# NVlabs/UnseenObjectClustering

Measured on AMD Instinct MI355X. Metric: frames/sec at 640x480 RGB-D, two-stage clustering, higher is better.
Workload: dtype f32; 1 GPU; configs[3] frames: full two-stage (crop-and-refine) segmentation of single 640x480 RGB-D frames; throughput schedule 3 streams x 4-frame launch sets (one frame at a time: `latency`); frame=640x480, seeds=100, iters=10, crop=224, total_frames=513, frames_per_gpu=513, collective=False, frames_in_flight_per_gpu=12, streams_per_gpu=3, frames_per_launch=4

## Files before the change

include/uoc_hip.h:

```cpp
#ifndef UOC_HIP_H
#define UOC_HIP_H

#include <stddef.h>
#include <stdint.h>

#ifdef __cplusplus
extern "C" {
#endif

#define UOC_OK 0
#define UOC_EINVAL (-22)
#define UOC_ENOMEM (-12)
#define UOC_EHIP (-5)
#define UOC_ENOENT (-2)
#define UOC_ETIMEDOUT (-110)

#define UOC_EMBED_DIM 64
#define UOC_MAX_SEEDS 128
#define UOC_METRIC_COSINE 0
#define UOC_METRIC_EUCLIDEAN 1

int uoc_version(void);
int uoc_is_dev_build(void);
unsigned long long uoc_config_fingerprint(void);
// ... 32 lines not shown
size_t uoc_ms_workspace_bytes_wide(int batch, int n, int m, int halves);
int uoc_ms_cluster_wide(const float *d_X, int halves, int batch, int n, int m, float kappa, int iters, float epsilon,
                        const int32_t *d_first_index, int32_t *d_labels, int32_t *d_indices, float *d_Z_out,
                        int32_t *d_seed_labels_out, void *d_ws, size_t ws_bytes, void *stream);

int uoc_ms_select_seeds_ex(const float *d_X, int batch, int n, int m, int num_init, const int32_t *d_first_index,
                           float *d_seeds, int32_t *d_indices, int metric, void *d_ws, size_t ws_bytes, void *stream);
int uoc_ms_hill_climb_ex(const float *d_X, int batch, int n, float *d_Z, int m, float kappa, int iters, int metric,
                         void *d_ws, size_t ws_bytes, void *stream);
int uoc_ms_seed_components_ex(const float *d_Z, int batch, int m, float epsilon, int metric, int32_t *d_seed_labels,
                              int32_t *d_num_unique, void *stream);
int uoc_ms_assign_ex(const float *d_X, int batch, int n, const float *d_Z, const int32_t *d_seed_labels,
                     const int32_t *d_num_unique, int m, int metric, int32_t *d_labels, int32_t *d_closest, void *d_ws,
                     size_t ws_bytes, void *stream);
int uoc_ms_cluster_ex(const float *d_X, int batch, int n, int m, float kappa, int iters, float epsilon, int metric,
                      const int32_t *d_first_index, int32_t *d_labels, int32_t *d_indices, float *d_Z_out,
                      int32_t *d_seed_labels_out, void *d_ws, size_t ws_bytes, void *stream);
int uoc_ms_cluster_wide_ex(const float *d_X, int halves, int batch, int n, int m, float kappa, int iters, float epsilon,
                           int metric, const int32_t *d_first_index, int32_t *d_labels, int32_t *d_indices, float *d_Z_out,
                           int32_t *d_seed_labels_out, void *d_ws, size_t ws_bytes, void *stream);


typedef struct uoc_net uoc_net;

enum { UOC_NET_RGBD_ADD = 0, UOC_NET_COLOR = 1, UOC_NET_DEPTH = 2, UOC_NET_RGBD_EARLY = 3, UOC_NET_RGBD_CAT = 4 };

int uoc_net_create(uoc_net **out);
int uoc_net_create_mode(uoc_net **out, int mode);
int uoc_net_embed_dim(const uoc_net *net);
int uoc_net_destroy(uoc_net *net);
int uoc_net_load_param(uoc_net *net, const char *name, const float *host_data, size_t numel);
int uoc_net_finalize(uoc_net *net);
size_t uoc_net_workspace_bytes(const uoc_net *net, int B, int H, int W);
int uoc_net_set_split_precision(uoc_net *net, int on);
int uoc_net_forward(uoc_net *net, const float *d_rgb, const float *d_xyz, int B, int H, int W, float *d_embed,
                    void *d_ws, size_t ws_bytes, void *stream);

#define UOC_CONV_DIRECT 0
#define UOC_CONV_WINOGRAD4 4
#define UOC_CONV_WINOGRAD4_BF16X3 5
int uoc_conv2d_nhwc(const float *d_in, const float *d_w, const float *d_bias, const float *d_res, float *d_out,
                    int G, int B, int H, int W, int Cin, int Cout, int K, int stride, int dil, int pad, int relu,
                    void *stream);
int uoc_conv2d_nhwc_algo(const float *d_in, const float *d_w, const float *d_bias, const float *d_res, float *d_out,
                         int G, int B, int H, int W, int Cin, int Cout, int K, int stride, int dil, int pad, int relu,
                         int algo, void *stream);

int uoc_conv2d_tile_list(int algo, int32_t *out_pairs, int cap);
int uoc_conv2d_nhwc_tile(const float *d_in, const float *d_w, const float *d_bias, const float *d_res, float *d_out,
                         int G, int B, int H, int W, int Cin, int Cout, int K, int stride, int dil, int pad, int relu,
                         int algo, void *stream, int cfg, int bm);
int uoc_conv2d_tile_choice(int G, int B, int H, int W, int Cin, int Cout, int K, int stride, int dil, int algo,
                           int32_t *cfg, int32_t *bm, int32_t *family_bm);
int uoc_net_stem(const float *d_nchw, const float *h_w, const float *h_bias, const float *d_res, int G, int B, int H,
                 int W, int relu, float *d_out, void *stream);
int uoc_maxpool3x3s2_nhwc(const float *d_in, float *d_out, int n_img, int H, int W, int C, void *stream);
int uoc_head(const float *d_fa, const float *d_fb, float *d_embed, int B, int h, int w, int H, int W, int cat,
             void *stream);


typedef struct uoc_roi_table {
  int32_t K;
  int32_t label[128];
  int32_t box[128][4];
} uoc_roi_table;

size_t uoc_roi_workspace_bytes(void);

int uoc_prep_rgbd(const uint8_t *d_bgr, const uint16_t *d_depth_mm, int H, int W, float fx, float fy, float px,
                  float py, float mean_b, float mean_g, float mean_r, float *d_image, float *d_xyz, void *stream);

int uoc_filter_labels_depth(int32_t *d_labels, const float *d_z, long z_batch_stride, int B, int H, int W,
                            float threshold, void *d_ws, size_t ws_bytes, void *stream);

int uoc_roi_build(int32_t *d_labels, const float *d_z, int H, int W, float threshold, float pad_fraction,
                  uoc_roi_table *d_table, void *d_ws, size_t ws_bytes, void *stream);

int uoc_roi_crop(const float *d_rgb, const float *d_xyz, const int32_t *d_labels, int H, int W,
                 const uoc_roi_table *d_table, int K, int S, float *d_rgb_crops, float *d_xyz_crops,
                 float *d_mask_crops, void *stream);

int uoc_roi_match_stats(const int32_t *d_labels_crop, const float *d_mask_crops, const float *d_xyz_crops, int K,
                        int S, int32_t *d_keep, float *d_meanz, void *d_ws, size_t ws_bytes, void *stream);

int uoc_roi_paste(const int32_t *d_labels_crop, const uoc_roi_table *d_table, const int32_t *d_map,
                  const int32_t *d_order, int K, int S, int H, int W, int32_t *d_refined, void *stream);

int uoc_roi_match(const int32_t *d_labels_crop, const float *d_mask_crops, const float *d_xyz_crops,
                  const uoc_roi_table *d_table, int K, int S, int H, int W, int32_t *d_refined, int32_t *d_keep,
                  int32_t *d_plan, int32_t *d_status, void *d_ws, size_t ws_bytes, void *stream);

int uoc_labels_to_u8(const int32_t *d_labels, long n, uint8_t *d_out, int32_t *d_top, void *stream);


typedef struct uoc_eval_tables {
  int32_t cont[128 * 128];
  int32_t prec_tp[128 * 128];
  int32_t rec_tp[128 * 128];
  int32_t bnd_pred[128];
  int32_t bnd_gt[128];
  int32_t bad_label;
} uoc_eval_tables;

size_t uoc_eval_workspace_bytes(int H, int W);
int uoc_eval_pair_stats(const int32_t *d_pred, const int32_t *d_gt, int H, int W, int radius, uoc_eval_tables *d_tables,
                        void *d_ws, size_t ws_bytes, void *stream);
// ... 207 lines not shown
```

unseenobjectclustering_amd/_native.py:

```python
from __future__ import annotations

import ctypes
import os
from ctypes import c_char_p, c_float, c_int, c_int32, c_size_t, c_void_p, POINTER

from .build import LIB_PATH

_lib = None


class NativeError(RuntimeError):
    pass


def _declare(lib):
    P = c_void_p
    lib.uoc_version.restype = c_int
    lib.uoc_is_dev_build.argtypes = []
    lib.uoc_is_dev_build.restype = c_int
    lib.uoc_config_fingerprint.argtypes = []
    lib.uoc_config_fingerprint.restype = ctypes.c_ulonglong
    lib.uoc_shutdown.restype = c_int
    lib.uoc_reload_env.argtypes = []
    lib.uoc_reload_env.restype = c_int
    lib.uoc_shutdown.argtypes = []
    lib.uoc_last_error.restype = c_char_p
    lib.uoc_ms_set_persistent_fps.argtypes = [c_int]
    lib.uoc_ms_set_persistent_fps.restype = c_int
    lib.uoc_ms_set_stream_ordering.argtypes = [c_int]
    lib.uoc_ms_set_stream_ordering.restype = c_int
    lib.uoc_ms_fps_fallbacks.argtypes = []
    lib.uoc_ms_fps_fallbacks.restype = c_int
    lib.uoc_ms_workspace_bytes.restype = c_size_t
    lib.uoc_ms_workspace_bytes.argtypes = [c_int, c_int, c_int]
    lib.uoc_ms_select_seeds.argtypes = [P, c_int, c_int, c_int, P, P, P, P, c_size_t, P]
    lib.uoc_ms_select_seeds_from.argtypes = [P, c_int, c_int, c_int, c_int, P, P, P, P, c_size_t, P]
    lib.uoc_ms_hill_climb.argtypes = [P, c_int, c_int, P, c_int, c_float, c_int, P, c_size_t, P]
    lib.uoc_ms_seed_components.argtypes = [P, c_int, c_int, c_float, P, P, P]
    lib.uoc_ms_assign.argtypes = [P, c_int, c_int, P, P, P, c_int, P, P, P, c_size_t, P]
    lib.uoc_ms_cluster.argtypes = [P, c_int, c_int, c_int, c_float, c_int, c_float, P, P, P, P, P, P, c_size_t, P]
    lib.uoc_ms_check.argtypes = [P]
    lib.uoc_ms_check.restype = c_int
    lib.uoc_ms_workspace_bytes_wide.restype = c_size_t
    lib.uoc_ms_workspace_bytes_wide.argtypes = [c_int, c_int, c_int, c_int]
    lib.uoc_ms_cluster_wide.argtypes = [P, c_int, c_int, c_int, c_int, c_float, c_int, c_float, P, P, P, P, P, P, c_size_t, P]
    lib.uoc_ms_cluster_wide.restype = c_int
    lib.uoc_ms_select_seeds_ex.argtypes = [P, c_int, c_int, c_int, c_int, P, P, P, c_int, P, c_size_t, P]
    lib.uoc_ms_hill_climb_ex.argtypes = [P, c_int, c_int, P, c_int, c_float, c_int, c_int, P, c_size_t, P]
    lib.uoc_ms_seed_components_ex.argtypes = [P, c_int, c_int, c_float, c_int, P, P, P]
    lib.uoc_ms_assign_ex.argtypes = [P, c_int, c_int, P, P, P, c_int, c_int, P, P, P, c_size_t, P]
    lib.uoc_ms_cluster_ex.argtypes = [P, c_int, c_int, c_int, c_float, c_int, c_float, c_int, P, P, P, P, P, P, c_size_t, P]
    lib.uoc_ms_cluster_wide_ex.argtypes = [P, c_int, c_int, c_int, c_int, c_float, c_int, c_float, c_int, P, P, P, P, P, P,
                                           c_size_t, P]
    for name in METRIC_SYMBOLS:
        getattr(lib, name).restype = c_int
    lib.uoc_net_embed_dim.argtypes = [P]
    lib.uoc_net_embed_dim.restype = c_int
    lib.uoc_net_create.argtypes = [POINTER(P)]
    lib.uoc_net_create_mode.argtypes = [POINTER(P), c_int]
    lib.uoc_net_destroy.argtypes = [P]
    lib.uoc_net_load_param.argtypes = [P, c_char_p, P, c_size_t]
    lib.uoc_net_finalize.argtypes = [P]
    lib.uoc_net_workspace_bytes.restype = c_size_t
    lib.uoc_net_workspace_bytes.argtypes = [P, c_int, c_int, c_int]
    lib.uoc_net_forward.argtypes = [P, P, P, c_int, c_int, c_int, P, P, c_size_t, P]
    lib.uoc_net_set_split_precision.argtypes = [P, c_int]
    lib.uoc_net_set_split_precision.restype = c_int
    lib.uoc_conv2d_nhwc.argtypes = [P, P, P, P, P] + [c_int] * 11 + [P]
    lib.uoc_conv2d_nhwc_algo.argtypes = [P, P, P, P, P] + [c_int] * 12 + [P]
    lib.uoc_conv2d_nhwc_algo.restype = c_int
    lib.uoc_conv2d_tile_list.argtypes = [c_int, P, c_int]
    lib.uoc_conv2d_nhwc_tile.argtypes = [P, P, P, P, P] + [c_int] * 12 + [P, c_int, c_int]
    lib.uoc_conv2d_tile_choice.argtypes = [c_int] * 10 + [P, P, P]
    lib.uoc_net_stem.argtypes = [P, P, P, P] + [c_int] * 5 + [P, P]
    lib.uoc_maxpool3x3s2_nhwc.argtypes = [P, P] + [c_int] * 4 + [P]
    lib.uoc_head.argtypes = [P, P, P] + [c_int] * 6 + [P]
    for name in TILE_SYMBOLS:
        getattr(lib, name).restype = c_int
    for name in ("uoc_net_create", "uoc_net_create_mode", "uoc_net_destroy", "uoc_net_load_param", "uoc_net_finalize", "uoc_net_forward",
                 "uoc_conv2d_nhwc"):
        getattr(lib, name).restype = c_int
    lib.uoc_eval_workspace_bytes.restype = c_size_t
    lib.uoc_eval_workspace_bytes.argtypes = [c_int, c_int]
    lib.uoc_eval_pair_stats.argtypes = [P, P, c_int, c_int, c_int, P, P, c_size_t, P]
    lib.uoc_eval_pair_stats.restype = c_int
    lib.uoc_roi_workspace_bytes.restype = c_size_t
    lib.uoc_roi_workspace_bytes.argtypes = []
    lib.uoc_prep_rgbd.argtypes = [P, P, c_int, c_int] + [c_float] * 7 + [P, P, P]
    lib.uoc_prep_rgbd.restype = c_int
    lib.uoc_filter_labels_depth.argtypes = [P, P, ctypes.c_long, c_int, c_int, c_int, c_float, P, c_size_t, P]
    lib.uoc_roi_build.argtypes = [P, P, c_int, c_int, c_float, c_float, P, P, c_size_t, P]
    lib.uoc_roi_crop.argtypes = [P, P, P, c_int, c_int, P, c_int, c_int, P, P, P, P]
    lib.uoc_roi_match_stats.argtypes = [P, P, P, c_int, c_int, P, P, P, c_size_t, P]
    lib.uoc_roi_paste.argtypes = [P, P, P, P, c_int, c_int, c_int, c_int, P, P]
    lib.uoc_labels_to_u8.argtypes = [P, ctypes.c_long, P, P, P]
    lib.uoc_roi_match.argtypes = [P, P, P, P, c_int, c_int, c_int, c_int, P, P, P, P, P, c_size_t, P]
    for name in ("uoc_filter_labels_depth", "uoc_roi_build", "uoc_roi_crop", "uoc_roi_match_stats", "uoc_roi_paste", "uoc_labels_to_u8", "uoc_roi_match"):
        getattr(lib, name).restype = c_int
    lib.uoc_objects_workspace_bytes.argtypes = [c_int, c_int, c_int]
    lib.uoc_objects_workspace_bytes.restype = c_size_t
    lib.uoc_objects.argtypes = [P, P, P, c_int, c_int, c_int, c_int, c_int, P, P, P, P, ctypes.c_long, P, P, c_size_t, P]
    lib.uoc_objects.restype = c_int
    lib.uoc_track_state_bytes.argtypes = [c_int, c_int, c_int]
    lib.uoc_track_state_bytes.restype = c_size_t
    lib.uoc_track_workspace_bytes.argtypes = [c_int]
    lib.uoc_track_workspace_bytes.restype = c_size_t
    lib.uoc_track_reset.argtypes = [P, c_int, c_int, c_int, c_int, P]
    lib.uoc_track_reset.restype = c_int
    lib.uoc_track_step.argtypes = [P, c_int, c_int, c_int, c_int, c_int, P, P, P, P, P, c_size_t, P]
    lib.uoc_track_step.restype = c_int
    lib.uoc_cc_workspace_bytes.argtypes = [c_int, c_int, c_int]
    lib.uoc_cc_workspace_bytes.restype = c_size_t
    lib.uoc_cc_split.argtypes = [P, c_int, c_int, c_int, c_int, c_int, c_int, P, P, P, P, c_size_t, P]
    lib.uoc_cc_split.restype = c_int
    lib.uoc_plane_workspace_bytes.argtypes = [c_int, c_int, c_int, c_int]
    lib.uoc_plane_workspace_bytes.restype = c_size_t
    lib.uoc_support_plane.argtypes = [P, P, c_int, c_int, c_int, c_int, c_int, ctypes.c_uint32, P, P, P, P, c_size_t, P]
    lib.uoc_support_plane.restype = c_int
    lib.uoc_planes_workspace_bytes.argtypes = [c_int, c_int, c_int, c_int, c_int]
    lib.uoc_planes_workspace_bytes.restype = c_size_t
    lib.uoc_support_planes.argtypes = [P, P] + [c_int] * 8 + [ctypes.c_uint32, P, P, P, P, P, P, c_size_t, P]
    lib.uoc_support_planes.restype = c_int
    lib.uoc_relations_workspace_bytes.argtypes = [c_int, c_int, c_int]
    lib.uoc_relations_workspace_bytes.restype = c_size_t
    lib.uoc_relations.argtypes = [P, P, c_int, c_int, c_int, c_int, c_int, c_int, P, P, P, c_size_t, P]
    lib.uoc_relations.restype = c_int
    lib.uoc_placement_workspace_bytes.argtypes = [c_int, c_int, c_int, c_int]
    lib.uoc_placement_workspace_bytes.restype = c_size_t
    lib.uoc_placement.argtypes = [P, P, P] + [c_int] * 9 + [P, c_int, P, P, P, P, P, P, P, c_size_t, P]
    lib.uoc_placement.restype = c_int
    lib.uoc_grasp_workspace_bytes.argtypes = [c_int, c_int, c_int, c_int]
    lib.uoc_grasp_workspace_bytes.restype = c_size_t
    lib.uoc_grasp.argtypes = [P, P, c_int, c_int, P] + [c_int] * 7 + [P, P, P, c_size_t, P]
    lib.uoc_grasp.restype = c_int
    lib.uoc_elevation_workspace_bytes.argtypes = [c_int, c_int, c_int, c_int]
    lib.uoc_elevation_workspace_bytes.restype = c_size_t
    lib.uoc_elevation.argtypes = [P, P, P] + [c_int] * 8 + [P, c_int] + [P] * 9 + [c_size_t, P]
    lib.uoc_elevation.restype = c_int
    lib.uoc_footprint_workspace_bytes.argtypes = [c_int, c_int, c_int, c_int]
    lib.uoc_footprint_workspace_bytes.restype = c_size_t
    lib.uoc_footprint.argtypes = [P, P, P, P, c_int, c_int, P, c_int, P, c_int, c_int, P, P, P, P, c_size_t, P]
    lib.uoc_footprint.restype = c_int
    lib.uoc_routes_workspace_bytes.argtypes = [c_int, c_int, c_int]
    lib.uoc_routes_workspace_bytes.restype = c_size_t
    lib.uoc_routes.argtypes = [P, P, P, c_int, c_int, P, c_int, c_int, c_int, P, P, P, P, c_size_t, P]
    lib.uoc_routes.restype = c_int
    lib.uoc_ms_confidence_workspace_bytes.argtypes = [c_int, c_int, c_int, c_int]
    lib.uoc_ms_confidence_workspace_bytes.restype = c_size_t
    lib.uoc_ms_confidence.argtypes = [P, c_int, c_int, c_int, P, P, P, c_int, c_int, P, P, P, P, P, P, c_size_t, P]
    lib.uoc_ms_confidence.restype = c_int
    lib.uoc_conf_paste.argtypes = [P, P, P, P, c_int, c_int, c_int, c_int, P, P]
    lib.uoc_conf_paste.restype = c_int
    lib.uoc_conf_objects.argtypes = [P, P, c_int, c_int, c_int, c_int, P, P]
    lib.uoc_conf_objects.restype = c_int
    lib.uoc_normals_workspace_bytes.argtypes = [c_int, c_int, c_int]
    lib.uoc_normals_workspace_bytes.restype = c_size_t
    lib.uoc_normals.argtypes = [P, P, P] + [c_int] * 7 + [P, c_int, c_int, c_int, P, P, P, P, c_size_t, P]
    lib.uoc_normals.restype = c_int
    lib.uoc_lzf_decompress.argtypes = [P, c_size_t, P, c_size_t]
    lib.uoc_lzf_decompress.restype = ctypes.c_long
    lib.uoc_prof_enable.argtypes = [c_int]
    lib.uoc_prof_reset.argtypes = []
    lib.uoc_prof_report.argtypes = [ctypes.c_char_p, c_size_t]
    for name in ("uoc_prof_enable", "uoc_prof_reset", "uoc_prof_report"):
        getattr(lib, name).restype = c_int
    for name in ("uoc_ms_select_seeds", "uoc_ms_select_seeds_from", "uoc_ms_hill_climb", "uoc_ms_seed_components", "uoc_ms_assign",
                 "uoc_ms_cluster"):
        getattr(lib, name).restype = c_int


METRIC_COSINE = 0
METRIC_EUCLIDEAN = 1
METRICS = {"cosine": METRIC_COSINE, "euclidean": METRIC_EUCLIDEAN}
METRIC_SYMBOLS = ("uoc_ms_select_seeds_ex", "uoc_ms_hill_climb_ex", "uoc_ms_seed_components_ex", "uoc_ms_assign_ex",
                  "uoc_ms_cluster_ex", "uoc_ms_cluster_wide_ex")


TILE_SYMBOLS = ("uoc_conv2d_tile_list", "uoc_conv2d_nhwc_tile", "uoc_conv2d_tile_choice", "uoc_net_stem",
                "uoc_maxpool3x3s2_nhwc", "uoc_head")


def metric_code(metric) -> int:
    if metric not in METRICS:
        raise NotImplementedError(f"metric={metric!r}: only 'cosine' and 'euclidean' are implemented on gfx950")
    return METRICS[metric]


EXPORTED_SYMBOLS = (
    "uoc_version", "uoc_is_dev_build", "uoc_config_fingerprint", "uoc_shutdown", "uoc_last_error", "uoc_reload_env", "uoc_ms_set_persistent_fps", "uoc_ms_set_stream_ordering", "uoc_ms_fps_fallbacks", "uoc_ms_check", "uoc_ms_workspace_bytes", "uoc_ms_select_seeds", "uoc_ms_select_seeds_from", "uoc_ms_hill_climb",
    "uoc_ms_seed_components", "uoc_ms_assign", "uoc_ms_cluster", "uoc_ms_workspace_bytes_wide", "uoc_ms_cluster_wide",
) + METRIC_SYMBOLS + (
    "uoc_net_embed_dim",
    "uoc_net_create", "uoc_net_create_mode", "uoc_net_destroy", "uoc_net_load_param", "uoc_net_finalize", "uoc_net_workspace_bytes",
    "uoc_net_forward", "uoc_net_set_split_precision", "uoc_conv2d_nhwc", "uoc_conv2d_nhwc_algo",
) + TILE_SYMBOLS + (
    "uoc_roi_workspace_bytes", "uoc_prep_rgbd", "uoc_filter_labels_depth", "uoc_roi_build", "uoc_roi_crop", "uoc_roi_match_stats",
    "uoc_roi_paste", "uoc_roi_match", "uoc_labels_to_u8", "uoc_eval_workspace_bytes", "uoc_eval_pair_stats", "uoc_objects_workspace_bytes", "uoc_objects",
    "uoc_track_state_bytes", "uoc_track_workspace_bytes", "uoc_track_reset", "uoc_track_step",
    "uoc_cc_workspace_bytes", "uoc_cc_split", "uoc_plane_workspace_bytes", "uoc_support_plane",
    "uoc_planes_workspace_bytes", "uoc_support_planes",
    "uoc_relations_workspace_bytes", "uoc_relations", "uoc_placement_workspace_bytes", "uoc_placement",
    "uoc_grasp_workspace_bytes", "uoc_grasp", "uoc_elevation_workspace_bytes", "uoc_elevation",
    "uoc_footprint_workspace_bytes", "uoc_footprint", "uoc_routes_workspace_bytes", "uoc_routes",
    "uoc_ms_confidence_workspace_bytes", "uoc_ms_confidence", "uoc_conf_paste", "uoc_conf_objects",
    "uoc_normals_workspace_bytes", "uoc_normals", "uoc_lzf_decompress", "uoc_prof_enable", "uoc_prof_reset", "uoc_prof_report",
)


class RoiTable(ctypes.Structure):
    _fields_ = [("K", c_int32), ("label", c_int32 * 128), ("box", (c_int32 * 4) * 128)]


ROI_TABLE_BYTES = ctypes.sizeof(RoiTable)


class UocObject(ctypes.Structure):
    _fields_ = [("pixels", c_int32), ("count", c_int32), ("box", c_int32 * 4), ("centroid", c_float * 3), ("cov", c_float * 6),
                ("aabb_min", c_float * 3), ("aabb_max", c_float * 3), ("eig", c_float * 3), ("axes", c_float * 9),
                ("obb_center", c_float * 3), ("obb_half", c_float * 3), ("offset", c_int32), ("kept", c_int32)]


OBJECT_BYTES = ctypes.sizeof(UocObject)


class UocPlane(ctypes.Structure):
    _fields_ = [("found", c_int32), ("candidates", c_int32), ("inliers", c_int32), ("hyp", c_int32), ("normal", c_float * 3),
                ("d", c_float), ("centroid", c_float * 3), ("eig", c_float * 3), ("rms", c_float), ("u", c_float * 3),
                ("v", c_float * 3)]


class UocPlaneObject(ctypes.Structure):
    _fields_ = [("count", c_int32), ("height_min", c_float), ("height_max", c_float), ("foot", c_float * 2),
# ... 173 lines not shown
```

unseenobjectclustering_amd/csrc/conv.h:

```cpp
#pragma once
#include "common.h"

namespace uoc {

struct ConvParams {
  const float *in;
  const float *w;
  const float *bias;
  const float *res;
  float *out;
  int G, B, H, W, Cin, Ho, Wo, Cout;
  int KH, KW, stride, dil, pad, relu;
  int stem;
  int tune = 1;
  int prof_kc = -1;
  double prof_flops = 0.0;
  int prof_tag[4] = {0, 0, 0, 0};
};

int launch_conv(const ConvParams &p, hipStream_t st);
int conv_tile_list(int *out_pairs, int cap);
int conv_tile_choice(const ConvParams &p, int *cfg, int *bm, int *fam_bm);
int launch_conv_tile(const ConvParams &p, hipStream_t st, int cfg, int bm);

struct W4Tile {
  int bm, bn;
};
int wino4_tile_list(bool split, int *out_pairs, int cap);
void wino4_tile_choice(bool split, int NT, int Cout, int planes, int *bn, int *bm);
int wino4_split_tile_list(int *out_pairs, int cap);
void wino4_split_tile_choice(int NT, int Cout, int planes, int *bn, int *bm);
void wino4_pick_tile(const int (*tiles)[2], int n, int NT, int Cout, int planes, int &bm, int &bn);
int wino4_plane_grid(int NT, int Cout, int planes, int bm, int bn);

bool wino4_eligible(const ConvParams &p);
bool wino4_channels_ok(int Cin, int Cout);
size_t wino4_ws_floats(int G, int B, int H, int W, int d, int Cin, int Cout);
int wino4_num_tiles(int B, int H, int W, int d);
int launch_wino4_weights(const float *w, float *U, int G, int Cout, int Cin, hipStream_t st);
int launch_wino4_conv(const ConvParams &p, const float *U, float *ws, hipStream_t st, const unsigned short *U3 = nullptr,
                      const W4Tile *tile = nullptr);
int launch_wino4_split_weights(const float *U, unsigned short *U3, int G, int Cout, int Cin, hipStream_t st);
int launch_wino4_slice_split(const ConvParams &p0, int Bg, int b0, const unsigned short *U3, float *ws, hipStream_t st,
                             const W4Tile *tile = nullptr);
struct Wino4Geom;
int w4_stage_output(const ConvParams &p, const Wino4Geom &geo, const float *Mw, hipStream_t st);
long wino4_elem_blocks(long items);
int launch_nchw3_to_nhwc4(const float *in, float *out, int B, int H, int W, hipStream_t st);
int launch_maxpool3x3s2(const float *in, float *out, int n_img, int H, int W, int C, int Ho, int Wo, hipStream_t st);
int launch_head(const float *fa, const float *fb, float *embed, int B, int h, int w, int H, int W, int cat,
                hipStream_t st);

}
```

unseenobjectclustering_amd/csrc/net.hip:

```cpp
#include <map>
#include <mutex>
#include <string>
#include <vector>

#include "conv.h"

#include <stdlib.h>

namespace uoc {

struct ConvLayer {
  std::string conv, bn;
  int Cin, Cout, K, stride, dil, pad, relu;
  bool has_bn, has_bias, stem;
  float *d_w = nullptr, *d_b = nullptr;
  float *d_U4 = nullptr;
  unsigned short *d_U3 = nullptr;
  size_t w_per_group = 0;
};

struct Block {
  int conv1, conv2, down;
};

// ... 352 lines not shown
    if (int rc = run_conv(G, c2, tmp, res, y, B, ho, wo, ho, wo, st, w.wino, n->split)) return rc;
    cur = (cur + 3) & 3;
    h = ho;
    wd = wo;
  }
  if (int rc = run_conv(G, n->layers[n->fc], w.buf[cur], nullptr, w.fc, B, h, wd, h, wd, st)) return rc;
  return launch_head(w.fc, G == 2 ? w.fc + (size_t)B * h * wd * 64 : nullptr, d_embed, B, h, wd, H, W,
                     n->mode == UOC_NET_RGBD_CAT, st);
}

static ConvParams entry_params(int G, int B, int H, int W, int Cin, int Cout, int K, int stride, int dil, int pad, int relu) {
  ConvParams p;
  p.tune = 0;
  p.in = p.w = p.bias = p.res = nullptr;
  p.out = nullptr;
  p.G = G;
  p.B = B;
  p.H = H;
  p.W = W;
  p.Cin = Cin;
  p.Cout = Cout;
  p.KH = p.KW = K;
  p.stride = stride;
  p.dil = dil;
  p.pad = pad;
  p.relu = relu;
  p.stem = 0;
  p.Ho = (H + 2 * pad - dil * (K - 1) - 1) / stride + 1;
  p.Wo = (W + 2 * pad - dil * (K - 1) - 1) / stride + 1;
  return p;
}

static int conv2d_entry(const float *d_in, const float *d_w, const float *d_bias, const float *d_res, float *d_out, int G,
                        int B, int H, int W, int Cin, int Cout, int K, int stride, int dil, int pad, int relu, int algo,
                        void *stream, const int *tile) {
  UOC_REQUIRE(K == 1 || K == 3, "K=%d (only 1 or 3)", K);
  UOC_REQUIRE(G >= 1 && B >= 1 && H >= 1 && W >= 1 && Cin >= 1 && Cout >= 1 && stride >= 1 && dil >= 1 && pad >= 0,
              "conv2d: bad shape");
  UOC_REQUIRE(d_res == nullptr || d_res != d_out, "conv2d: the residual must not alias the output");
  ConvParams p = entry_params(G, B, H, W, Cin, Cout, K, stride, dil, pad, relu);
  p.in = d_in;
  p.w = d_w;
  p.bias = d_bias;
  p.res = d_res;
  p.out = d_out;
  hipStream_t st = (hipStream_t)stream;
  if (algo == UOC_CONV_DIRECT) return tile ? launch_conv_tile(p, st, tile[0], tile[1]) : launch_conv(p, st);
  const W4Tile w4tile = {tile ? tile[1] : 0, tile ? tile[0] : 0};
  const W4Tile *wt = tile ? &w4tile : nullptr;
  static std::mutex mu;
  std::lock_guard<std::mutex> lock(mu);
  if (algo == UOC_CONV_WINOGRAD4 || algo == UOC_CONV_WINOGRAD4_BF16X3) {
    UOC_REQUIRE(wino4_eligible(p), "conv2d: shape not eligible for Winograd F(4x4,3x3)");
    if (tile) {
      int pairs[2 * 32];
      const int n = wino4_tile_list(algo == UOC_CONV_WINOGRAD4_BF16X3, pairs, 32);
      bool listed = false;
      for (int i = 0; i < n && i < 32; ++i) listed = listed || (pairs[2 * i] == tile[0] && pairs[2 * i + 1] == tile[1]);
      UOC_REQUIRE(listed, "conv2d tile: the plane GEMM has no tile BN=%d BM=%d", tile[0], tile[1]);
      UOC_REQUIRE(Cout % tile[0] == 0, "conv2d tile: Cout=%d is not a multiple of BN=%d", Cout, tile[0]);
    }
    static float *U4 = nullptr, *ws4 = nullptr;
    static unsigned short *U3 = nullptr;
    static size_t ucap4 = 0, wcap4 = 0, ucap3 = 0;
    const size_t un = (size_t)G * 36 * Cout * Cin, wn = wino4_ws_floats(G, B, H, W, dil, Cin, Cout);
    if (un > ucap4) {
      if (U4) (void)hipFree(U4);
      UOC_HIP_CHECK(hipMalloc(&U4, un * sizeof(float)));
      ucap4 = un;
    }
    if (wn > wcap4) {
      if (ws4) (void)hipFree(ws4);
      UOC_HIP_CHECK(hipMalloc(&ws4, wn * sizeof(float)));
      wcap4 = wn;
    }
    if (int rc = launch_wino4_weights(d_w, U4, G, Cout, Cin, st)) return rc;
    if (algo == UOC_CONV_WINOGRAD4_BF16X3) {
      if (3 * un > ucap3) {
        if (U3) (void)hipFree(U3);
        UOC_HIP_CHECK(hipMalloc(&U3, 3 * un * sizeof(unsigned short)));
        ucap3 = 3 * un;
      }
      if (int rc = launch_wino4_split_weights(U4, U3, G, Cout, Cin, st)) return rc;
      return launch_wino4_conv(p, U4, ws4, st, U3, wt);
    }
    return launch_wino4_conv(p, U4, ws4, st, nullptr, wt);
  }
  set_error("conv2d: unknown algorithm %d", algo);
  return UOC_EINVAL;
}

int uoc_conv2d_nhwc_algo(const float *d_in, const float *d_w, const float *d_bias, const float *d_res, float *d_out, int G,
                         int B, int H, int W, int Cin, int Cout, int K, int stride, int dil, int pad, int relu, int algo,
                         void *stream) {
  return conv2d_entry(d_in, d_w, d_bias, d_res, d_out, G, B, H, W, Cin, Cout, K, stride, dil, pad, relu, algo, stream, nullptr);
}

int uoc_conv2d_nhwc_tile(const float *d_in, const float *d_w, const float *d_bias, const float *d_res, float *d_out, int G,
                         int B, int H, int W, int Cin, int Cout, int K, int stride, int dil, int pad, int relu, int algo,
                         void *stream, int cfg, int bm) {
  UOC_REQUIRE(d_in && d_w && d_out, "conv2d tile: null pointer");
  const int tile[2] = {cfg, bm};
  return conv2d_entry(d_in, d_w, d_bias, d_res, d_out, G, B, H, W, Cin, Cout, K, stride, dil, pad, relu, algo, stream, tile);
}

int uoc_conv2d_tile_list(int algo, int32_t *out_pairs, int cap) {
  UOC_REQUIRE(cap >= 0 && (out_pairs || cap == 0), "tile list: null array");
  if (algo == UOC_CONV_DIRECT) return conv_tile_list(out_pairs, cap);
  if (algo == UOC_CONV_WINOGRAD4 || algo == UOC_CONV_WINOGRAD4_BF16X3)
    return wino4_tile_list(algo == UOC_CONV_WINOGRAD4_BF16X3, out_pairs, cap);
  set_error("tile list: unknown algorithm %d", algo);
  return UOC_EINVAL;
}

int uoc_conv2d_tile_choice(int G, int B, int H, int W, int Cin, int Cout, int K, int stride, int dil, int algo, int32_t *cfg,
                           int32_t *bm, int32_t *family_bm) {
  UOC_REQUIRE(cfg && bm, "tile choice: null pointer");
  UOC_REQUIRE(K == 1 || K == 3, "K=%d (only 1 or 3)", K);
  UOC_REQUIRE(G >= 1 && B >= 1 && H >= 1 && W >= 1 && Cin >= 1 && Cout >= 1 && stride >= 1 && dil >= 1, "tile choice: bad shape");
  const ConvParams p = entry_params(G, B, H, W, Cin, Cout, K, stride, dil, K == 3 ? dil : 0, 0);
  if (algo == UOC_CONV_DIRECT) return conv_tile_choice(p, cfg, bm, family_bm);
  if (algo == UOC_CONV_WINOGRAD4 || algo == UOC_CONV_WINOGRAD4_BF16X3) {
    UOC_REQUIRE(wino4_eligible(p), "tile choice: shape not eligible for Winograd F(4x4,3x3)");
    int bn_ = 0, bm_ = 0;
    wino4_tile_choice(algo == UOC_CONV_WINOGRAD4_BF16X3, wino4_num_tiles(B, H, W, dil), Cout, 36 * G, &bn_, &bm_);
    *cfg = bn_;
    *bm = bm_;
    return UOC_OK;
  }
  set_error("tile choice: unknown algorithm %d", algo);
  return UOC_EINVAL;
}

int uoc_net_stem(const float *d_nchw, const float *h_w, const float *h_bias, const float *d_res, int G, int B, int H, int W,
                 int relu, float *d_out, void *stream) {
  UOC_REQUIRE(d_nchw && h_w && d_out, "stem: null pointer");
  UOC_REQUIRE(G >= 1 && B >= 1 && H >= 1 && W >= 1, "stem: bad shape");
  UOC_REQUIRE(d_res == nullptr || d_res != d_out, "stem: the residual must not alias the output");
  UOC_REQUIRE((long)G * B * H * W * 4 < (1l << 31), "stem: input too large");
  hipStream_t st = (hipStream_t)stream;
  const size_t wpg = (size_t)7 * 64 * 32;
  std::vector<float> hw((size_t)G * wpg, 0.f), hb((size_t)G * 64, 0.f);
  const std::vector<double> one(64, 1.0);
  for (int g = 0; g < G; ++g) relayout_weights(h_w + (size_t)g * 64 * 3 * 49, one.data(), 64, 3, 7, true, wpg, hw.data() + g * wpg);
  if (h_bias) hb.assign(h_bias, h_bias + (size_t)G * 64);
  float *d_w = nullptr, *d_b = nullptr, *d_in4 = nullptr;
  int rc = UOC_OK;
  auto run = [&]() -> int {
    UOC_HIP_CHECK(hipMalloc(&d_w, hw.size() * sizeof(float)));
    UOC_HIP_CHECK(hipMalloc(&d_b, hb.size() * sizeof(float)));
    UOC_HIP_CHECK(hipMalloc(&d_in4, (size_t)G * B * H * W * 4 * sizeof(float)));
    UOC_HIP_CHECK(hipMemcpyAsync(d_w, hw.data(), hw.size() * sizeof(float), hipMemcpyHostToDevice, st));
    UOC_HIP_CHECK(hipMemcpyAsync(d_b, hb.data(), hb.size() * sizeof(float), hipMemcpyHostToDevice, st));
    if (int r = launch_nchw3_to_nhwc4(d_nchw, d_in4, G * B, H, W, st)) return r;
    ConvLayer L;
    L.Cin = 3;
// ... 46 lines not shown
```

unseenobjectclustering_amd/csrc/wino4.hip:

```cpp
#include "conv.h"
#include "dma.h"
#include "prof.h"
#include "wino4_math.h"

#include <stdlib.h>

namespace uoc {

constexpr int W4BK = 32;
#ifndef W4_OUT_MIN_BLOCKS
#define W4_OUT_MIN_BLOCKS 2
#endif

__global__ __launch_bounds__(256) void wino4_weight_kernel(const float *__restrict__ w, float *__restrict__ U, int G,
                                                           int Cout, int Cin) {
  const long total = (long)G * Cout * Cin;
  for (long i = (long)blockIdx.x * blockDim.x + threadIdx.x; i < total; i += (long)gridDim.x * blockDim.x) {
    const int ci = (int)(i % Cin);
    const int co = (int)((i / Cin) % Cout);
    const int g = (int)(i / ((long)Cin * Cout));
    wino4_weight_body(w, U, G, Cout, Cin, g, co, ci);
  }
}

// ... 314 lines not shown
  const size_t lds = (size_t)NSTAGE * (BM + BN) * W4BK * sizeof(float);
  static_assert((size_t)NSTAGE * (BM + BN) * W4BK * sizeof(float) <= 160 * 1024, "LDS ring too large");
  UOC_REQUIRE(!PAIR || (Cin / W4BK) % 2 == 0, "winograd F(4x4): the pair loop needs an even number of 32-channel chunks");
  static DeviceOnce attr_set;
  if (!attr_set.done()) {
    UOC_HIP_CHECK(hipFuncSetAttribute(reinterpret_cast<const void *>(&wino4_gemm_kernel<BM, BN, PAIR, NW>),
                                      hipFuncAttributeMaxDynamicSharedMemorySize, (int)lds));
    attr_set.mark();
  }
  hipLaunchKernelGGL((wino4_gemm_kernel<BM, BN, PAIR, NW>), dim3(nblocks), dim3(NW * 64), lds, st, V, U, Mo, NT, Cin, Cout, planes,
                     mtiles, nt_shift);
  UOC_LAUNCH_CHECK();
  return UOC_OK;
}

#define UOC_W4_TILES(X) \
  X(96, 128) X(128, 128) X(160, 128) X(192, 128) X(96, 64) X(128, 64) X(160, 64) X(192, 64)
static const int kW4Tiles[][2] = {
#define X(A, B) {A, B},
    UOC_W4_TILES(X)
#undef X
};

static int plane_per_xcd() {
  const int dev = device_num_cu(), ncu = dev > 0 ? dev : 256;
  return ncu / 8 > 0 ? ncu / 8 : 1;
}

void wino4_pick_tile(const int (*tiles)[2], int n, int NT, int Cout, int planes, int &bm, int &bn) {
  const int per_xcd = plane_per_xcd();
  double best = -1;
  for (int i = 0; i < n; ++i) {
    const int BM = tiles[i][0], BN = tiles[i][1];
    if (Cout % BN) continue;
    const long items = (long)planes * ((NT + BM - 1) / BM) * (Cout / BN);
    const long S = (items + 7) / 8;
    const long steps = (S + per_xcd - 1) / per_xcd;
    const double cost = (double)steps * BM * BN * (1.0 + 0.05 * (192.0 / BM - 1.0)) * (BN == 64 ? 1.06 : 1.0);
    if (best < 0 || cost < best) {
      best = cost;
      bm = BM;
      bn = BN;
    }
  }
}

int wino4_plane_grid(int NT, int Cout, int planes, int bm, int bn) {
  const int per_xcd = plane_per_xcd();
  const long items = (long)planes * ((NT + bm - 1) / bm) * (Cout / bn);
  const long S = (items + 7) / 8;
  return 8 * (int)(S < per_xcd ? S : per_xcd);
}

static int launch_wino4_gemm(const float *V, const float *U, float *Mo, int NT, int Cin, int Cout, int planes, hipStream_t st,
                             const W4Tile *tile) {
  int bm = 160, bn = Cout % 128 == 0 ? 128 : 64;
  if (tile) {
    bm = tile->bm;
    bn = tile->bn;
    UOC_REQUIRE((bn == 64 || bn == 128) && Cout % bn == 0, "winograd F(4x4): Cout=%d does not admit BN=%d", Cout, bn);
  } else {
    wino4_pick_tile(kW4Tiles, (int)(sizeof(kW4Tiles) / sizeof(kW4Tiles[0])), NT, Cout, planes, bm, bn);
  }
  const int nblocks = wino4_plane_grid(NT, Cout, planes, bm, bn);
  const int cpt = Cin / W4BK;
  const bool pair = cpt % 2 == 0 && cpt >= 4;
#define X(A, B)                                                                                                      \
  if (bm == A && bn == B)                                                                                            \
    return pair ? launch_wino4_gemm_t<A, B, true, 8>(V, U, Mo, NT, Cin, Cout, planes, nblocks, st)                    \
                : launch_wino4_gemm_t<A, B, false, 8>(V, U, Mo, NT, Cin, Cout, planes, nblocks, st);
  UOC_W4_TILES(X)
#undef X
  set_error("winograd F(4x4): no GEMM tile %dx%d", bm, bn);
  return UOC_EINVAL;
}

int wino4_tile_list(bool split, int *out_pairs, int cap) {
  if (split) return wino4_split_tile_list(out_pairs, cap);
  const int n = (int)(sizeof(kW4Tiles) / sizeof(kW4Tiles[0]));
  for (int i = 0; i < n && i < cap && out_pairs; ++i) {
    out_pairs[2 * i] = kW4Tiles[i][1];
    out_pairs[2 * i + 1] = kW4Tiles[i][0];
  }
  return n;
}

void wino4_tile_choice(bool split, int NT, int Cout, int planes, int *bn, int *bm) {
  if (split) return wino4_split_tile_choice(NT, Cout, planes, bn, bm);
  *bm = 160;
  *bn = Cout % 128 == 0 ? 128 : 64;
  wino4_pick_tile(kW4Tiles, (int)(sizeof(kW4Tiles) / sizeof(kW4Tiles[0])), NT, Cout, planes, *bm, *bn);
}

bool wino4_channels_ok(int Cin, int Cout) {
  const int n64 = Cout / 64;
  return Cin % W4BK == 0 && Cout % 64 == 0 && n64 > 0 && (n64 & (n64 - 1)) == 0;
}

bool wino4_eligible(const ConvParams &p) {
  return !p.stem && p.KH == 3 && p.KW == 3 && p.stride == 1 && p.pad == p.dil && wino4_channels_ok(p.Cin, p.Cout) &&
         p.Ho == p.H && p.Wo == p.W;
}

int wino4_num_tiles(int B, int H, int W, int d) { return make_geom4(B, H, W, d).NT; }

size_t wino4_ws_floats(int G, int B, int H, int W, int d, int Cin, int Cout) {
  const Wino4Geom geo = make_geom4(B, H, W, d);
  return (size_t)G * 36 * geo.NT * 5 / 2 * (size_t)(Cin > Cout ? Cin : Cout) + 64;
// ... 92 lines not shown
```

Baseline: 176.7 frames/s.

## Add streaming plane GEMM for Winograd F(4x4) with weights resident in LDS

Adds a new Winograd transform-domain GEMM kernel for Cin=Cout=64 and 128. Each block keeps a Cout slice of U in LDS, and its waves stream 16-row groups of V, double-buffering the next rows in registers and storing results with buffer stores. The kernel is selected by default whenever the channel class matches. The grid is planned from CU count and residency so planes split into row ranges across CUs. It aims to replace the generic tiled GEMM for these common shapes with one that reuses weights better and has a simpler schedule, at the risk of lower efficiency for some plane counts.

```diff
diff --git a/include/uoc_hip.h b/include/uoc_hip.h
--- a/include/uoc_hip.h
+++ b/include/uoc_hip.h
@@ -108,6 +108,9 @@
                          int algo, void *stream, int cfg, int bm);
 int uoc_conv2d_tile_choice(int G, int B, int H, int W, int Cin, int Cout, int K, int stride, int dil, int algo,
                            int32_t *cfg, int32_t *bm, int32_t *family_bm);
+int uoc_conv2d_nhwc_wino4_stream(const float *d_in, const float *d_w, const float *d_bias, const float *d_res, float *d_out,
+                                 int G, int B, int H, int W, int Cin, int Cout, int dil, int relu, void *stream);
+int uoc_wino4_stream_plan(int planes, int rows, int Cin, int Cout, int num_cu, int32_t *plan, int32_t *blocks, int cap);
 int uoc_net_stem(const float *d_nchw, const float *h_w, const float *h_bias, const float *d_res, int G, int B, int H,
                  int W, int relu, float *d_out, void *stream);
 int uoc_maxpool3x3s2_nhwc(const float *d_in, float *d_out, int n_img, int H, int W, int C, void *stream);
diff --git a/unseenobjectclustering_amd/_native.py b/unseenobjectclustering_amd/_native.py
--- a/unseenobjectclustering_amd/_native.py
+++ b/unseenobjectclustering_amd/_native.py
@@ -72,6 +72,8 @@
     lib.uoc_conv2d_tile_list.argtypes = [c_int, P, c_int]
     lib.uoc_conv2d_nhwc_tile.argtypes = [P, P, P, P, P] + [c_int] * 12 + [P, c_int, c_int]
     lib.uoc_conv2d_tile_choice.argtypes = [c_int] * 10 + [P, P, P]
+    lib.uoc_conv2d_nhwc_wino4_stream.argtypes = [P, P, P, P, P] + [c_int] * 8 + [P]
+    lib.uoc_wino4_stream_plan.argtypes = [c_int] * 5 + [P, P, c_int]
     lib.uoc_net_stem.argtypes = [P, P, P, P] + [c_int] * 5 + [P, P]
     lib.uoc_maxpool3x3s2_nhwc.argtypes = [P, P] + [c_int] * 4 + [P]
     lib.uoc_head.argtypes = [P, P, P] + [c_int] * 6 + [P]
@@ -176,8 +178,8 @@
                   "uoc_ms_cluster_ex", "uoc_ms_cluster_wide_ex")
 
 
-TILE_SYMBOLS = ("uoc_conv2d_tile_list", "uoc_conv2d_nhwc_tile", "uoc_conv2d_tile_choice", "uoc_net_stem",
-                "uoc_maxpool3x3s2_nhwc", "uoc_head")
+TILE_SYMBOLS = ("uoc_conv2d_tile_list", "uoc_conv2d_nhwc_tile", "uoc_conv2d_tile_choice", "uoc_conv2d_nhwc_wino4_stream",
+                "uoc_wino4_stream_plan", "uoc_net_stem", "uoc_maxpool3x3s2_nhwc", "uoc_head")
 
 
 def metric_code(metric) -> int:
diff --git a/unseenobjectclustering_amd/csrc/conv.h b/unseenobjectclustering_amd/csrc/conv.h
--- a/unseenobjectclustering_amd/csrc/conv.h
+++ b/unseenobjectclustering_amd/csrc/conv.h
@@ -33,6 +33,22 @@
 void wino4_pick_tile(const int (*tiles)[2], int n, int NT, int Cout, int planes, int &bm, int &bn);
 int wino4_plane_grid(int NT, int Cout, int planes, int bm, int bn);
 
+constexpr int W4_STREAM = -1;
+struct W4StreamPlan {
+  int grid;
+  int units;
+  int ranges;
+  int ngroups;
+  int nslices;
+  int wn;
+  int nw;
+  int lds;
+  int bound;
+};
+bool wino4_stream_admits(int Cin, int Cout);
+bool wino4_stream_plan(int planes, int NT, int Cin, int Cout, int ncu, W4StreamPlan *plan);
+bool wino4_stream_block(const W4StreamPlan &plan, int block, int *plane, int *slice, int *lo, int *hi);
+
 bool wino4_eligible(const ConvParams &p);
 bool wino4_channels_ok(int Cin, int Cout);
 size_t wino4_ws_floats(int G, int B, int H, int W, int d, int Cin, int Cout);
diff --git a/unseenobjectclustering_amd/csrc/net.hip b/unseenobjectclustering_amd/csrc/net.hip
--- a/unseenobjectclustering_amd/csrc/net.hip
+++ b/unseenobjectclustering_amd/csrc/net.hip
@@ -428,7 +428,11 @@
   std::lock_guard<std::mutex> lock(mu);
   if (algo == UOC_CONV_WINOGRAD4 || algo == UOC_CONV_WINOGRAD4_BF16X3) {
     UOC_REQUIRE(wino4_eligible(p), "conv2d: shape not eligible for Winograd F(4x4,3x3)");
-    if (tile) {
+    const bool stream = tile && tile[0] == W4_STREAM && tile[1] == W4_STREAM;
+    if (stream) {
+      UOC_REQUIRE(algo == UOC_CONV_WINOGRAD4 && wino4_stream_admits(Cin, Cout),
+                  "conv2d: the streaming plane GEMM does not take Cin=%d Cout=%d", Cin, Cout);
+    } else if (tile) {
       int pairs[2 * 32];
       const int n = wino4_tile_list(algo == UOC_CONV_WINOGRAD4_BF16X3, pairs, 32);
       bool listed = false;
@@ -476,8 +480,33 @@
                          int B, int H, int W, int Cin, int Cout, int K, int stride, int dil, int pad, int relu, int algo,
                          void *stream, int cfg, int bm) {
   UOC_REQUIRE(d_in && d_w && d_out, "conv2d tile: null pointer");
+  UOC_REQUIRE(cfg != W4_STREAM || bm != W4_STREAM, "conv2d tile: no tile BN=%d BM=%d", cfg, bm);
   const int tile[2] = {cfg, bm};
   return conv2d_entry(d_in, d_w, d_bias, d_res, d_out, G, B, H, W, Cin, Cout, K, stride, dil, pad, relu, algo, stream, tile);
+}
+
+int uoc_conv2d_nhwc_wino4_stream(const float *d_in, const float *d_w, const float *d_bias, const float *d_res, float *d_out, int G,
+                                 int B, int H, int W, int Cin, int Cout, int dil, int relu, void *stream) {
+  UOC_REQUIRE(d_in && d_w && d_out, "conv2d stream: null pointer");
+  const int tile[2] = {W4_STREAM, W4_STREAM};
+  return conv2d_entry(d_in, d_w, d_bias, d_res, d_out, G, B, H, W, Cin, Cout, 3, 1, dil, dil, relu, UOC_CONV_WINOGRAD4, stream, tile);
+}
+
+int uoc_wino4_stream_plan(int planes, int rows, int Cin, int Cout, int num_cu, int32_t *plan, int32_t *blocks, int cap) {
+  UOC_REQUIRE(planes >= 1 && rows >= 1 && Cin >= 1 && Cout >= 1 && cap >= 0 && (blocks || cap == 0), "stream plan: bad argument");
+  W4StreamPlan sp;
+  if (!wino4_stream_plan(planes, rows, Cin, Cout, num_cu, &sp)) return 0;
+  if (plan) {
+    const int32_t v[8] = {sp.grid, sp.nslices, sp.ranges, sp.ngroups, sp.wn, sp.nw, sp.lds, sp.bound};
+    for (int i = 0; i < 8; ++i) plan[i] = v[i];
+  }
+  for (int b = 0; b < sp.grid && b < cap; ++b) {
+    int pl = -1, sl = -1, lo = 0, hi = 0;
+    if (!wino4_stream_block(sp, b, &pl, &sl, &lo, &hi)) pl = sl = -1, lo = hi = 0;
+    const int32_t v[4] = {pl, sl, lo, hi};
+    for (int i = 0; i < 4; ++i) blocks[4 * b + i] = v[i];
+  }
+  return 1;
 }
 
 int uoc_conv2d_tile_list(int algo, int32_t *out_pairs, int cap) {
diff --git a/unseenobjectclustering_amd/csrc/wino4.hip b/unseenobjectclustering_amd/csrc/wino4.hip
--- a/unseenobjectclustering_amd/csrc/wino4.hip
+++ b/unseenobjectclustering_amd/csrc/wino4.hip
@@ -390,8 +390,169 @@
   return 8 * (int)(S < per_xcd ? S : per_xcd);
 }
 
+__host__ __device__ inline bool w4s_block(int block, int units, int nslices, int ranges, int ngroups, int &plane, int &slice,
+                                          int &lo, int &hi) {
+  const int eight = block >> 3;
+  slice = eight % nslices;
+  const int u = (eight / nslices) * 8 + (block & 7);
+  if (u >= units) return false;
+  plane = u / ranges;
+  const int r = u - plane * ranges;
+  lo = (int)((long)ngroups * r / ranges);
+  hi = (int)((long)ngroups * (r + 1) / ranges);
+  return true;
+}
+
+typedef unsigned w4s_u32x4 __attribute__((ext_vector_type(4)));
+
+template <int CIN, int WN, int NW>
+__global__ __launch_bounds__(NW * 64, 4) void wino4_stream_kernel(const float *__restrict__ V, const float *__restrict__ U,
+                                                                  float *__restrict__ Mo, int NT, int Cout, int ranges,
+                                                                  int ngroups, int nslices, int units) {
+  constexpr int NF = CIN / 16, TN = WN / 16;
+  extern __shared__ __attribute__((aligned(16))) float4 w4s_u[];
+  int plane, slice, lo, hi;
+  if (!w4s_block(blockIdx.x, units, nslices, ranges, ngroups, plane, slice, lo, hi)) return;
+  const int tid = threadIdx.x, lane = tid & 63;
+  const int wave = __builtin_amdgcn_readfirstlane(tid >> 6);
+  const int t = lane & 15, q = lane >> 4;
+  const float *Vp = V + (size_t)plane * NT * CIN + 4 * q;
+  const float *Up = U + ((size_t)plane * Cout + (size_t)slice * WN) * CIN;
+  const __amdgpu_buffer_rsrc_t srd_m =
+      __builtin_amdgcn_make_buffer_rsrc(Mo + (size_t)plane * NT * Cout, 0, (int)((unsigned)NT * (unsigned)Cout * 4u), 0x00020000);
+  const unsigned row_bytes = (unsigned)Cout * 4u, col_bytes = ((unsigned)slice * WN + 4 * q) * 4u;
+
+  auto rows = [&](int g) { return reinterpret_cast<const float4 *>(Vp + (size_t)min(16 * g + t, NT - 1) * CIN); };
+  int g = lo + wave;
+  float4 xb[NF];
+  if (g < hi) {
+    const float4 *src = rows(g);
+#pragma unroll
+    for (int f = 0; f < NF; ++f) xb[f] = src[4 * f];
+  }
+  constexpr int NFILL = NF * TN / NW;
+  static_assert(NF * TN % NW == 0, "U fragments per wave");
+  {
+    float4 uf[NFILL];
+#pragma unroll
+    for (int k = 0; k < NFILL; ++k) {
+      const int fj = k * NW + wave, j = fj % TN, f = fj / TN;
+      uf[k] = *reinterpret_cast<const float4 *>(Up + (size_t)(16 * j + t) * CIN + 16 * f + 4 * q);
+    }
+#pragma unroll
+    for (int k = 0; k < NFILL; ++k) w4s_u[(k * NW + wave) * 64 + lane] = uf[k];
+  }
+  __syncthreads();
+
+  constexpr int JB = TN < 4 ? TN : 4, NH = TN / JB, NS = NF * NH;
+  static_assert(TN % JB == 0 && NS % 2 == 0, "step count");
+  float4 wa[2][JB];
+#pragma unroll
+  for (int j = 0; j < JB; ++j) wa[0][j] = w4s_u[j * 64 + lane];
+  for (; g < hi; g += NW) {
+    const float4 *nxt = rows(g + NW < hi ? g + NW : g);
+    f32x4 acc[TN];
+#pragma unroll
+    for (int j = 0; j < TN; ++j) acc[j] = f32x4{0.f, 0.f, 0.f, 0.f};
+    float4 x, xn[NF];
+#pragma unroll
+    for (int f = 0; f < NF; ++f) xn[f] = nxt[4 * f];
+#pragma unroll
+    for (int s = 0; s < NS; ++s) {
+      const int f = s / NH, j0 = (s % NH) * JB, sn = (s + 1) % NS;
+#pragma unroll
+      for (int j = 0; j < JB; ++j) wa[(s + 1) & 1][j] = w4s_u[((sn / NH) * TN + (sn % NH) * JB + j) * 64 + lane];
+      if (s % NH == 0) x = xb[f];
+#pragma unroll
+      for (int j = 0; j < JB; ++j) acc[j0 + j] = w4mfma(wa[s & 1][j].x, x.x, acc[j0 + j]);
+#pragma unroll
+      for (int j = 0; j < JB; ++j) acc[j0 + j] = w4mfma(wa[s & 1][j].y, x.y, acc[j0 + j]);
+#pragma unroll
+      for (int j = 0; j < JB; ++j) acc[j0 + j] = w4mfma(wa[s & 1][j].z, x.z, acc[j0 + j]);
+#pragma unroll
+      for (int j = 0; j < JB; ++j) acc[j0 + j] = w4mfma(wa[s & 1][j].w, x.w, acc[j0 + j]);
+      __builtin_amdgcn_sched_barrier(0);
+    }
+    const unsigned voff = (unsigned)(16 * g + t) * row_bytes + col_bytes;
+#pragma unroll
+    for (int j = 0; j < TN; ++j) __builtin_amdgcn_raw_buffer_store_b128(__builtin_bit_cast(w4s_u32x4, acc[j]), srd_m, (int)(voff + 64 * j), 0, 0);
+#pragma unroll
+    for (int f = 0; f < NF; ++f) xb[f] = xn[f];
+  }
+}
+
+struct W4StreamClass {
+  int cin, cout, wn, nw, per_cu;
+};
+static const W4StreamClass kW4Stream[] = {
+    {64, 64, 64, 4, 4},
+    {128, 128, 64, 4, 4},
+};
+
+static const W4StreamClass *w4s_class(int Cin, int Cout) {
+  for (const W4StreamClass &c : kW4Stream)
+    if (c.cin == Cin && c.cout == Cout) return &c;
+  return nullptr;
+}
+
+bool wino4_stream_admits(int Cin, int Cout) { return w4s_class(Cin, Cout) != nullptr; }
+
+bool wino4_stream_plan(int planes, int NT, int Cin, int Cout, int ncu, W4StreamPlan *plan) {
+  const W4StreamClass *c = w4s_class(Cin, Cout);
+  if (!c) return false;
+  if (ncu <= 0) ncu = device_num_cu();
+  if (ncu <= 0) ncu = 256;
+  plan->ngroups = (NT + 15) / 16;
+  plan->nslices = Cout / c->wn;
+  plan->wn = c->wn;
+  plan->nw = c->nw;
+  plan->lds = Cin * c->wn * (int)sizeof(float);
+  const long resident = (long)ncu * c->per_cu / plan->nslices;
+  long ranges = resident / planes;
+  const long most = (plan->ngroups + c->nw - 1) / c->nw;
+  ranges = ranges < most ? ranges : most;
+  plan->ranges = (int)(ranges > 1 ? ranges : 1);
+  plan->units = planes * plan->ranges;
+  plan->grid = (plan->units + 7) / 8 * 8 * plan->nslices;
+  const long most_units = planes > resident ? planes : resident;
+  plan->bound = (int)((most_units + 7) / 8 * 8 * plan->nslices);
+  return true;
+}
+
+bool wino4_stream_block(const W4StreamPlan &plan, int block, int *plane, int *slice, int *lo, int *hi) {
+  return w4s_block(block, plan.units, plan.nslices, plan.ranges, plan.ngroups, *plane, *slice, *lo, *hi);
+}
+
+template <int CIN, int WN, int NW>
+static int launch_wino4_stream_t(const float *V, const float *U, float *Mo, int NT, int Cout, int planes, const W4StreamPlan &plan,
+                                 hipStream_t st) {
+  static DeviceOnce attr_set;
+  if (!attr_set.done()) {
+    UOC_HIP_CHECK(hipFuncSetAttribute(reinterpret_cast<const void *>(&wino4_stream_kernel<CIN, WN, NW>),
+                                      hipFuncAttributeMaxDynamicSharedMemorySize, plan.lds));
+    attr_set.mark();
+  }
+  hipLaunchKernelGGL((wino4_stream_kernel<CIN, WN, NW>), dim3(plan.grid), dim3(NW * 64), plan.lds, st, V, U, Mo, NT, Cout,
+                     plan.ranges, plan.ngroups, plan.nslices, plan.units);
+  UOC_LAUNCH_CHECK();
+  return UOC_OK;
+}
+
+static int launch_wino4_stream(const float *V, const float *U, float *Mo, int NT, int Cin, int Cout, int planes, hipStream_t st) {
+  W4StreamPlan plan;
+  UOC_REQUIRE(wino4_stream_plan(planes, NT, Cin, Cout, 0, &plan), "winograd F(4x4): no streaming plane GEMM for Cin=%d Cout=%d", Cin,
+              Cout);
+  UOC_REQUIRE(NT >= 1 && ((size_t)NT + 16) * Cout * 4 < (1ull << 32), "winograd F(4x4): a plane of M exceeds 4 GB");
+  if (Cin == 64 && plan.wn == 64 && plan.nw == 4) return launch_wino4_stream_t<64, 64, 4>(V, U, Mo, NT, Cout, planes, plan, st);
+  if (Cin == 128 && plan.wn == 64 && plan.nw == 4) return launch_wino4_stream_t<128, 64, 4>(V, U, Mo, NT, Cout, planes, plan, st);
+  set_error("winograd F(4x4): streaming class Cin=%d wn=%d nw=%d has no instantiation", Cin, plan.wn, plan.nw);
+  return UOC_EINVAL;
+}
+
 static int launch_wino4_gemm(const float *V, const float *U, float *Mo, int NT, int Cin, int Cout, int planes, hipStream_t st,
                              const W4Tile *tile) {
+  if (tile ? tile->bm == W4_STREAM && tile->bn == W4_STREAM : wino4_stream_admits(Cin, Cout))
+    return launch_wino4_stream(V, U, Mo, NT, Cin, Cout, planes, st);
   int bm = 160, bn = Cout % 128 == 0 ? 128 : 64;
   if (tile) {
     bm = tile->bm;
```

After: 177.0 frames/s, median of 2. Within noise of the previous version (+0.2%).
